# Edresson/VoiceSplit

Hardware: AMD Instinct MI355X
Metric: utterances/sec (3 s clips, B=64/GPU) fwd+bwd, channels-last bf16 activations / tape, bf16 MFMA, fp32 accumulate / statistics / master weights (higher is better)
Workload: dtype bf16 (conv activations and tape stored as bf16; bf16 MFMA operands in the convs, the LSTM / head contractions and the BPTT, f16 operands in the forward recurrence; fp32 accumulate, BatchNorm statistics, gate arithmetic / cell state, loss head, master weights)

## Files before the change

voicesplit_amd/csrc/nhwc_edge.hip:

```cpp
#include "vs_internal.h"

namespace {

typedef unsigned u4v __attribute__((ext_vector_type(4)));
typedef unsigned u2v __attribute__((ext_vector_type(2)));

__device__ __forceinline__ float bf_lo(unsigned u) { return __uint_as_float(u << 16); }
__device__ __forceinline__ float bf_hi(unsigned u) { return __uint_as_float(u & 0xffff0000u); }

template <int NV>
__device__ __forceinline__ void fold_channel_sums(float (&v)[NV][8], double* __restrict__ stats, float* lds ,
                                                  unsigned* turn = nullptr) {
  const int lane = threadIdx.x & 63, wave = threadIdx.x >> 6;
#pragma unroll
  for (int q = 0; q < NV; ++q)
#pragma unroll
    for (int j = 0; j < 8; ++j) {
      float s = v[q][j];
      s += __shfl_xor(s, 8, 64);
      s += __shfl_xor(s, 16, 64);
      s += __shfl_xor(s, 32, 64);
      if (lane < 8) lds[(wave * NV + q) * 64 + lane * 8 + j] = s;
    }
  __syncthreads();
// ... 264 lines not shown
    for (int q = 0; q < 4; ++q) {
      const float z0 = bf_lo(v[q]), z1 = bf_hi(v[q]);
      const float d0 = bf_lo(g[q]) * nhwc_act_grad<ACT>(fmaf(z0, sc[2 * q], sh[2 * q]));
      const float d1 = bf_hi(g[q]) * nhwc_act_grad<ACT>(fmaf(z1, sc[2 * q + 1], sh[2 * q + 1]));
      o[q] = vs_pack_bf16(fmaf(cA[2 * q], d0, fmaf(cB[2 * q], z0, cC[2 * q])),
                          fmaf(cA[2 * q + 1], d1, fmaf(cB[2 * q + 1], z1, cC[2 * q + 1])));
    }
    return o;
  };
  long long i = (long long)blockIdx.x * 256 + threadIdx.x;
  for (; i + stride < npieces; i += 2 * stride) {
    const u4v g0 = __builtin_nontemporal_load(da + i), v0 = __builtin_nontemporal_load(z + i);
    const u4v g1 = __builtin_nontemporal_load(da + i + stride), v1 = __builtin_nontemporal_load(z + i + stride);
    __builtin_nontemporal_store(apply(g0, v0), dz + i);
    __builtin_nontemporal_store(apply(g1, v1), dz + i + stride);
  }
  if (i < npieces) __builtin_nontemporal_store(apply(__builtin_nontemporal_load(da + i), __builtin_nontemporal_load(z + i)), dz + i);
}

template <int ACT>
__global__ __launch_bounds__(256)
void nhwc_bn_bwd_first_kernel(const u4v* __restrict__ da, const u4v* __restrict__ z, const float* __restrict__ x,
                              long long npix, int F, const float* __restrict__ scale, const float* __restrict__ shift,
                              const float* __restrict__ coef, double* __restrict__ acc_out ) {
  __shared__ float red[4 * 7 * 64];
  const int piece = threadIdx.x & 7;
  float sc[8], sh[8], cA[8], cB[8], cC[8], acc[7][8];
#pragma unroll
  for (int j = 0; j < 8; ++j) {
    const int c = piece * 8 + j;
    sc[j] = scale[c]; sh[j] = shift[c]; cA[j] = coef[c]; cB[j] = coef[64 + c]; cC[j] = coef[128 + c];
#pragma unroll
    for (int k = 0; k < 7; ++k) acc[k][j] = 0.f;
  }
  const long long stride = (long long)gridDim.x * 32;
  const int sr = (int)(stride % F);
  long long p = (long long)blockIdx.x * 32 + (threadIdx.x >> 3);
  int f = (int)(p % F);
  for (; p < npix; p += stride, f += sr) {
    if (f >= F) f -= F;
    float xv[7];
    gather_x7(x + (p - f), f, F, piece, xv);
    const u4v g = __builtin_nontemporal_load(da + p * 8 + piece), v = __builtin_nontemporal_load(z + p * 8 + piece);
#pragma unroll
    for (int q = 0; q < 4; ++q) {
#pragma unroll
      for (int e = 0; e < 2; ++e) {
        const int j = 2 * q + e;
        const float zv = e ? bf_hi(v[q]) : bf_lo(v[q]);
        const float dy = (e ? bf_hi(g[q]) : bf_lo(g[q])) * nhwc_act_grad<ACT>(fmaf(zv, sc[j], sh[j]));
        const float dzv = fmaf(cA[j], dy, fmaf(cB[j], zv, cC[j]));
#pragma unroll
        for (int k = 0; k < 7; ++k) acc[k][j] = fmaf(dzv, xv[k], acc[k][j]);
      }
    }
  }
  const int lane = threadIdx.x & 63, wave = threadIdx.x >> 6;
#pragma unroll
  for (int k = 0; k < 7; ++k)
#pragma unroll
    for (int j = 0; j < 8; ++j) {
      float s = acc[k][j];
      s += __shfl_xor(s, 8, 64);
      s += __shfl_xor(s, 16, 64);
      s += __shfl_xor(s, 32, 64);
      if (lane < 8) red[(wave * 7 + k) * 64 + lane * 8 + j] = s;
    }
  __syncthreads();
  for (int i = threadIdx.x; i < 7 * 64; i += 256) {
    const int k = i / 64, c = i - k * 64;
    atomicAdd(acc_out + c * 7 + k, (double)(red[(0 * 7 + k) * 64 + c] + red[(1 * 7 + k) * 64 + c] + red[(2 * 7 + k) * 64 + c] + red[(3 * 7 + k) * 64 + c]));
  }
}

__global__ void nhwc_cvt_f64_f32_kernel(const double* __restrict__ src, float* __restrict__ dst, int n) {
  const int i = blockIdx.x * blockDim.x + threadIdx.x;
  if (i < n) dst[i] = (float)src[i];
}

struct LastBwdBn {
  const u4v* z;
  const float *scale, *shift, *mean, *invstd;
  double* stats;
  unsigned* turn;
};

template <int ACT>
__device__ __forceinline__ void nhwc_act_both(float y, float& a, float& d) {
  if (ACT == VS_ACT_MISH) {
    const float u = __builtin_amdgcn_exp2f(fminf(y, 20.0f) * 1.44269504088896340736f);
    const float n = u * (u + 2.0f);
    const float r = __builtin_amdgcn_rcpf(n + 2.0f);
    a = y * (n * r);
    const float dd = r * fmaf(4.0f * y * r, u * (u + 1.0f), n);
    d = y > 20.0f ? 1.0f : dd;
  } else if (ACT == VS_ACT_RELU) {
    a = fmaxf(y, 0.0f);
    d = y > 0.0f ? 1.0f : 0.0f;
  } else {
    a = y;
    d = 1.0f;
  }
}

template <int ACT>
__device__ __forceinline__ void nhwc_act_both2(vs_f32x2 y, vs_f32x2& a, vs_f32x2& d) {
  if (ACT == VS_ACT_MISH) {
    const vs_f32x2 yc = {fminf(y.x, 20.0f), fminf(y.y, 20.0f)};
    const vs_f32x2 e = yc * 1.44269504088896340736f;
    const vs_f32x2 u = {__builtin_amdgcn_exp2f(e.x), __builtin_amdgcn_exp2f(e.y)};
    const vs_f32x2 n = u * (u + 2.0f);
    const vs_f32x2 dn = n + 2.0f;
    const vs_f32x2 r = {__builtin_amdgcn_rcpf(dn.x), __builtin_amdgcn_rcpf(dn.y)};
    a = y * (n * r);
    d = r * __builtin_elementwise_fma((yc * 4.0f) * r, __builtin_elementwise_fma(u, u, u), n);
  } else if (ACT == VS_ACT_RELU) {
    a = vs_f32x2{fmaxf(y.x, 0.0f), fmaxf(y.y, 0.0f)};
    d = vs_f32x2{y.x > 0.0f ? 1.0f : 0.0f, y.y > 0.0f ? 1.0f : 0.0f};
  } else {
    a = y;
    d = vs_f32x2{1.0f, 1.0f};
  }
}

template <int DYACT, bool RECOMP = false>
__global__ __launch_bounds__(256)
void nhwc_conv_last_bwd_kernel(const float* __restrict__ dz8, const float* __restrict__ w, const u4v* __restrict__ a7,
                               u4v* __restrict__ din, float* __restrict__ part, long long npix, int F, LastBwdBn bn) {
  __shared__ float red[4 * 8 * 64];
  const int piece = threadIdx.x & 7;
  vs_f32x2 wr[8][4], acc[8][4];
  vs_f32x2 sc[4], sh[4], mu[4], is[4], bacc[2][4];
#pragma unroll
  for (int co = 0; co < 8; ++co)
#pragma unroll
    for (int q = 0; q < 4; ++q) {
      wr[co][q] = vs_f32x2{w[co * 64 + piece * 8 + 2 * q], w[co * 64 + piece * 8 + 2 * q + 1]};
      acc[co][q] = vs_f32x2{0.f, 0.f};
    }
  if (DYACT >= 0) {
#pragma unroll
    for (int q = 0; q < 4; ++q) {
      const int c = piece * 8 + 2 * q;
      sc[q] = vs_f32x2{bn.scale[c], bn.scale[c + 1]}; sh[q] = vs_f32x2{bn.shift[c], bn.shift[c + 1]};
      mu[q] = vs_f32x2{bn.mean[c], bn.mean[c + 1]}; is[q] = vs_f32x2{bn.invstd[c], bn.invstd[c + 1]};
      bacc[0][q] = vs_f32x2{0.f, 0.f}; bacc[1][q] = vs_f32x2{0.f, 0.f};
    }
  }
  const long long stride = (long long)gridDim.x * 32;
  const int sr = (int)(stride % F);
  const long long sq = stride / F;
  long long p = (long long)blockIdx.x * 32 + (threadIdx.x >> 3);
  long long row = p / F;
  int f = (int)(p - row * F);
  struct In { float d[8]; u4v zv, av; };
  auto fetch = [&](long long pq, long long rq, int fq, In& in) {
    const float* dzr = dz8 + rq * 8 * F + fq;
#pragma unroll
    for (int co = 0; co < 8; ++co) in.d[co] = dzr[(size_t)co * F];
    if (DYACT >= 0) in.zv = __builtin_nontemporal_load(bn.z + pq * 8 + piece);
    if (!RECOMP) in.av = __builtin_nontemporal_load(a7 + pq * 8 + piece);
  };
  In cur, nxt;
  cur.zv = cur.av = nxt.zv = nxt.av = u4v{0u, 0u, 0u, 0u};
  if (p < npix) fetch(p, row, f, cur);
  for (; p < npix; p += stride) {
    int fn = f + sr;
    long long rown = row + sq;
    if (fn >= F) { fn -= F; ++rown; }
    const long long pn = p + stride;
    if (pn < npix) fetch(pn, rown, fn, nxt);
    vs_f32x2 zf[4], dact[4];
    u4v av = cur.av;
    if (DYACT >= 0) {
#pragma unroll
      for (int q = 0; q < 4; ++q) {
        zf[q] = vs_f32x2{bf_lo(cur.zv[q]), bf_hi(cur.zv[q])};
        vs_f32x2 aq;
        nhwc_act_both2<(DYACT >= 0 ? DYACT : VS_ACT_NONE)>(__builtin_elementwise_fma(zf[q], sc[q], sh[q]), aq, dact[q]);
        if (RECOMP) av[q] = vs_pack_bf16(aq.x, aq.y);
      }
    }
    vs_f32x2 g[4];
#pragma unroll
    for (int q = 0; q < 4; ++q) g[q] = vs_f32x2{0.f, 0.f};
#pragma unroll
    for (int co = 0; co < 8; ++co) {
      const vs_f32x2 dd = {cur.d[co], cur.d[co]};
#pragma unroll
      for (int q = 0; q < 4; ++q) {
        g[q] = __builtin_elementwise_fma(wr[co][q], dd, g[q]);
        acc[co][q] = __builtin_elementwise_fma(dd, vs_f32x2{bf_lo(av[q]), bf_hi(av[q])}, acc[co][q]);
      }
    }
    if (DYACT >= 0) {
#pragma unroll
      for (int q = 0; q < 4; ++q) {
        g[q] *= dact[q];
        bacc[0][q] += g[q];
        bacc[1][q] = __builtin_elementwise_fma(g[q], (zf[q] - mu[q]) * is[q], bacc[1][q]);
      }
    }
    __builtin_nontemporal_store(u4v{vs_pack_bf16(g[0].x, g[0].y), vs_pack_bf16(g[1].x, g[1].y), vs_pack_bf16(g[2].x, g[2].y), vs_pack_bf16(g[3].x, g[3].y)},
                                din + p * 8 + piece);
    cur = nxt;
    f = fn;
    row = rown;
  }
  if (DYACT >= 0) {
    float b8[2][8];
#pragma unroll
    for (int q = 0; q < 4; ++q) {
      b8[0][2 * q] = bacc[0][q].x; b8[0][2 * q + 1] = bacc[0][q].y;
      b8[1][2 * q] = bacc[1][q].x; b8[1][2 * q + 1] = bacc[1][q].y;
    }
    fold_channel_sums<2>(b8, bn.stats, red, bn.turn);
    __syncthreads();
  }
  const int lane = threadIdx.x & 63, wave = threadIdx.x >> 6;
#pragma unroll
  for (int co = 0; co < 8; ++co)
#pragma unroll
    for (int j = 0; j < 8; ++j) {
      float s = (j & 1) ? acc[co][j >> 1].y : acc[co][j >> 1].x;
      s += __shfl_xor(s, 8, 64);
      s += __shfl_xor(s, 16, 64);
      s += __shfl_xor(s, 32, 64);
      if (lane < 8) red[(wave * 8 + co) * 64 + lane * 8 + j] = s;
    }
  __syncthreads();
  for (int i = threadIdx.x; i < 512; i += 256)
    part[(size_t)blockIdx.x * 512 + i] = red[i] + red[512 + i] + red[1024 + i] + red[1536 + i];
}

constexpr int kMomN = 7 + 28;

__global__ __launch_bounds__(256)
void nhwc_first_moments_kernel(const float* __restrict__ x, long long npix, int F, double* __restrict__ mom, unsigned* turn) {
  __shared__ float red[4][kMomN];
  float acc[kMomN];
#pragma unroll
  for (int i = 0; i < kMomN; ++i) acc[i] = 0.f;
  const long long stride = (long long)gridDim.x * 256;
  for (long long p = (long long)blockIdx.x * 256 + threadIdx.x; p < npix; p += stride) {
    const int f = (int)(p % F);
    const float* xr = x + (p - f);
    float xv[7];
#pragma unroll
    for (int k = 0; k < 7; ++k) {
      const int ff = f + k - 3;
      xv[k] = (ff >= 0 && ff < F) ? xr[ff] : 0.f;
    }
    int i = 7;
#pragma unroll
    for (int k = 0; k < 7; ++k) {
      acc[k] += xv[k];
#pragma unroll
      for (int k2 = k; k2 < 7; ++k2) { acc[i] = fmaf(xv[k], xv[k2], acc[i]); ++i; }
    }
  }
  const int lane = threadIdx.x & 63, wave = threadIdx.x >> 6;
#pragma unroll
  for (int i = 0; i < kMomN; ++i) {
    float v = acc[i];
#pragma unroll
    for (int o = 32; o > 0; o >>= 1) v += __shfl_xor(v, o, 64);
    if (lane == 0) red[wave][i] = v;
  }
  __syncthreads();
  const unsigned slot = blockIdx.x % VS_BN_STAT_SLOTS, rank_in_slot = blockIdx.x / VS_BN_STAT_SLOTS;
  unsigned* my_turn = turn ? turn + VS_TURN_SLOT + slot : nullptr;
  if (turn) mom += (size_t)slot * 64;
  vs_turn_begin(my_turn, rank_in_slot);
  if (threadIdx.x < kMomN) atomicAdd(mom + threadIdx.x, (double)red[0][threadIdx.x] + (double)red[1][threadIdx.x] + (double)red[2][threadIdx.x] + (double)red[3][threadIdx.x]);
  vs_turn_end(my_turn, rank_in_slot, (gridDim.x - slot + VS_BN_STAT_SLOTS - 1) / VS_BN_STAT_SLOTS);
}

__global__ void fold_moment_slots_kernel(const double* __restrict__ slots, double* __restrict__ mom) {
  if (threadIdx.x >= kMomN) return;
  double v = 0.0;
  for (int k = 0; k < VS_BN_STAT_SLOTS; ++k) v += slots[(size_t)k * 64 + threadIdx.x];
  mom[threadIdx.x] = v;
}

__device__ __forceinline__ double mom_R(const double* mom, int k, int k2) {
  if (k > k2) { const int t = k; k = k2; k2 = t; }
  return mom[7 + k * 7 - k * (k - 1) / 2 + (k2 - k)];
}

__global__ void nhwc_first_stats_kernel(const double* __restrict__ mom, const float* __restrict__ w, const float* __restrict__ bias,
                                        double count, double* __restrict__ stats) {
  const int c = threadIdx.x;
  if (c >= 64) return;
  const double b = bias[c];
  double ws = 0.0, q = 0.0;
  for (int k = 0; k < 7; ++k) {
    ws += (double)w[c * 7 + k] * mom[k];
    for (int k2 = 0; k2 < 7; ++k2) q += (double)w[c * 7 + k] * (double)w[c * 7 + k2] * mom_R(mom, k, k2);
  }
  stats[2 * c] = ws + count * b;
  stats[2 * c + 1] = q + 2.0 * b * ws + count * b * b;
}

template <int ACT>
__device__ __forceinline__ vs_f32x2 nhwc_act_grad2(vs_f32x2 y) {
  if (ACT == VS_ACT_RELU) return vs_f32x2{y.x > 0.f ? 1.f : 0.f, y.y > 0.f ? 1.f : 0.f};
  if (ACT == VS_ACT_MISH) {
    const vs_f32x2 yc = {fminf(y.x, 20.0f), fminf(y.y, 20.0f)};
    const vs_f32x2 e = yc * 1.44269504088896340736f;
    const vs_f32x2 u = {__builtin_amdgcn_exp2f(e.x), __builtin_amdgcn_exp2f(e.y)};
    const vs_f32x2 n = u * (u + 2.0f);
    const vs_f32x2 d = n + 2.0f;
    const vs_f32x2 r = {__builtin_amdgcn_rcpf(d.x), __builtin_amdgcn_rcpf(d.y)};
    const vs_f32x2 t = __builtin_elementwise_fma(u, u, u);
    return r * __builtin_elementwise_fma((yc * 4.0f) * r, t, n);
  }
  return vs_f32x2{1.f, 1.f};
}

template <int ACT>
__global__ __launch_bounds__(256)
void nhwc_first_bwd_kernel(const u4v* __restrict__ da, const float* __restrict__ x, const float* __restrict__ w, const float* __restrict__ bias,
                           long long npix, int F, const float* __restrict__ scale, const float* __restrict__ shift,
                           const float* __restrict__ mean, const float* __restrict__ invstd, double* __restrict__ acc_out ,
                           unsigned* turn) {
  __shared__ float red[4 * 9 * 64];
  const int piece = threadIdx.x & 7;
  vs_f32x2 wr[4][7], bs[4], sc[4], sh[4], mu[4], is[4], acc[9][4];
#pragma unroll
  for (int q = 0; q < 4; ++q) {
    const int c0 = piece * 8 + 2 * q;
    bs[q] = vs_f32x2{bias[c0], bias[c0 + 1]};
    sc[q] = vs_f32x2{scale[c0], scale[c0 + 1]};
    sh[q] = vs_f32x2{shift[c0], shift[c0 + 1]};
    mu[q] = vs_f32x2{mean[c0], mean[c0 + 1]};
    is[q] = vs_f32x2{invstd[c0], invstd[c0 + 1]};
#pragma unroll
    for (int k = 0; k < 7; ++k) wr[q][k] = vs_f32x2{w[c0 * 7 + k], w[(c0 + 1) * 7 + k]};
#pragma unroll
    for (int k = 0; k < 9; ++k) acc[k][q] = vs_f32x2{0.f, 0.f};
  }
  const long long stride = (long long)gridDim.x * 32;
  const int sr = (int)(stride % F);
  long long p = (long long)blockIdx.x * 32 + (threadIdx.x >> 3);
  int f = (int)(p % F);
  auto process = [&](float mine, const u4v& g) {
    float xv[7];
    exchange_x7(mine, xv);
#pragma unroll
    for (int q = 0; q < 4; ++q) {
      vs_f32x2 zv = bs[q];
#pragma unroll
      for (int k = 0; k < 7; ++k) zv = __builtin_elementwise_fma(wr[q][k], vs_f32x2{xv[k], xv[k]}, zv);
      const vs_f32x2 dy = vs_f32x2{bf_lo(g[q]), bf_hi(g[q])} * nhwc_act_grad2<ACT>(__builtin_elementwise_fma(zv, sc[q], sh[q]));
      acc[0][q] += dy;
      acc[1][q] = __builtin_elementwise_fma(dy, (zv - mu[q]) * is[q], acc[1][q]);
#pragma unroll
      for (int k = 0; k < 7; ++k) acc[2 + k][q] = __builtin_elementwise_fma(dy, vs_f32x2{xv[k], xv[k]}, acc[2 + k][q]);
    }
  };
  float mine = 0.f;
  u4v g = {0u, 0u, 0u, 0u};
  if (p < npix) {
    mine = load_x7(x + (p - f), f, F, piece);
    g = __builtin_nontemporal_load(da + p * 8 + piece);
  }
  for (; p < npix; p += stride) {
    int fn = f + sr;
    if (fn >= F) fn -= F;
    const long long pn = p + stride;
    float mine_next = 0.f;
    u4v g_next = {0u, 0u, 0u, 0u};
    if (pn < npix) {
      mine_next = load_x7(x + (pn - fn), fn, F, piece);
      g_next = __builtin_nontemporal_load(da + pn * 8 + piece);
    }
    process(mine, g);
    mine = mine_next;
    g = g_next;
    f = fn;
  }
  const int lane = threadIdx.x & 63, wave = threadIdx.x >> 6;
#pragma unroll
  for (int k = 0; k < 9; ++k)
#pragma unroll
    for (int j = 0; j < 8; ++j) {
      float s = (j & 1) ? acc[k][j >> 1].y : acc[k][j >> 1].x;
      s += __shfl_xor(s, 8, 64);
      s += __shfl_xor(s, 16, 64);
      s += __shfl_xor(s, 32, 64);
      if (lane < 8) red[(wave * 9 + k) * 64 + lane * 8 + j] = s;
    }
  __syncthreads();
  const unsigned slot = blockIdx.x % VS_BN_STAT_SLOTS, rank_in_slot = blockIdx.x / VS_BN_STAT_SLOTS;
  unsigned* my_turn = turn ? turn + VS_TURN_SLOT + slot : nullptr;
  double* dst = turn ? acc_out + (size_t)slot * 576 : acc_out;
  vs_turn_begin(my_turn, rank_in_slot);
  for (int i = threadIdx.x; i < 9 * 64; i += 256) {
    const int k = i / 64, c = i - k * 64;
    atomicAdd(dst + c * 9 + k, (double)(red[(0 * 9 + k) * 64 + c] + red[(1 * 9 + k) * 64 + c] + red[(2 * 9 + k) * 64 + c] + red[(3 * 9 + k) * 64 + c]));
  }
  vs_turn_end(my_turn, rank_in_slot, (gridDim.x - slot + VS_BN_STAT_SLOTS - 1) / VS_BN_STAT_SLOTS);
}

__global__ void fold_slots_f64_kernel(const double* __restrict__ slots, int nslots, int n, double* __restrict__ out) {
  const int i = blockIdx.x * blockDim.x + threadIdx.x;
  if (i >= n) return;
  double v = 0.0;
  for (int k = 0; k < nslots; ++k) v += slots[(size_t)k * n + i];
  out[i] = v;
}

__global__ void nhwc_first_bwd_finalize_kernel(const double* __restrict__ acc , const double* __restrict__ mom,
                                               const float* __restrict__ w, const float* __restrict__ bias, const float* __restrict__ scale,
                                               const float* __restrict__ mean, const float* __restrict__ invstd, double count, int train,
                                               float* __restrict__ dgamma, float* __restrict__ dbeta, float* __restrict__ dbias, float* __restrict__ dw) {
  const int c = threadIdx.x;
  if (c >= 64) return;
  const double sdy = acc[c * 9], sdyx = acc[c * 9 + 1];
  dgamma[c] = (float)sdyx;
  dbeta[c] = (float)sdy;
  const double cA = scale[c];
  double cB = 0.0, cC = 0.0;
  if (train) {
    cB = -cA * (double)invstd[c] * sdyx / count;
    cC = -cA * sdy / count - cB * (double)mean[c];
  }
  dbias[c] = train ? 0.f : (float)(cA * sdy);
  const double b = bias[c];
  for (int k = 0; k < 7; ++k) {
    double zx = b * mom[k];
    for (int k2 = 0; k2 < 7; ++k2) zx += (double)w[c * 7 + k2] * mom_R(mom, k2, k);
    dw[c * 7 + k] = (float)(cA * acc[c * 9 + 2 + k] + cB * zx + cC * mom[k]);
  }
}

int stream_blocks(long long items_per_block_sweep, long long total, long long cap = 2048) {
  long long nb = (total + items_per_block_sweep - 1) / items_per_block_sweep;
  if (nb > cap) nb = cap;
  return nb < 1 ? 1 : (int)nb;
}
int stream_blocks_wide(long long items_per_block_sweep, long long total) {
  long long nb = (total + items_per_block_sweep - 1) / items_per_block_sweep;
  if (nb > (1LL << 24)) nb = 1LL << 24;
  return nb < 1 ? 1 : (int)nb;
}

}

int vs_nhwc_conv_first_impl(const float* x, const float* w, const float* scale, const float* shift, void* out,
                            int B, int T, int F, int act, double* bn_stats, hipStream_t stream, const float* bias) {
  VS_REQUIRE(x && w && scale && shift && out, "nhwc conv_first: NULL argument");
  VS_REQUIRE(B > 0 && T > 0 && F > 0, "nhwc conv_first: bad shape");
  const long long npix = (long long)B * T * F;
  const dim3 grid(stream_blocks(32, npix, (bn_stats && g_vs_turn) ? 2048 : 8192)), block(256);
  unsigned short* o = reinterpret_cast<unsigned short*>(out);
  if (bn_stats) {
    VS_REQUIRE(act == VS_ACT_NONE, "nhwc conv_first: fused statistics go with no activation");
    hipLaunchKernelGGL((nhwc_conv_first_kernel<VS_ACT_NONE, true>), grid, block, 0, stream, x, w, scale, shift, o, npix, F, bn_stats, bias);
  } else if (act == VS_ACT_NONE) hipLaunchKernelGGL((nhwc_conv_first_kernel<VS_ACT_NONE, false>), grid, block, 0, stream, x, w, scale, shift, o, npix, F, nullptr, bias);
  else if (act == VS_ACT_MISH) hipLaunchKernelGGL((nhwc_conv_first_kernel<VS_ACT_MISH, false>), grid, block, 0, stream, x, w, scale, shift, o, npix, F, nullptr, bias);
  else if (act == VS_ACT_RELU) hipLaunchKernelGGL((nhwc_conv_first_kernel<VS_ACT_RELU, false>), grid, block, 0, stream, x, w, scale, shift, o, npix, F, nullptr, bias);
  else VS_REQUIRE(false, "nhwc conv_first: unsupported activation %d", act);
  VS_LAUNCH_CHECK();
  return 0;
}

int vs_nhwc_first_moments_impl(const float* x, int B, int T, int F, double* mom, hipStream_t stream, double* det_slots, int mom_is_zero) {
  VS_REQUIRE(x && mom && B > 0 && T > 0 && F > 0, "nhwc first_moments: bad argument");
  const long long npix = (long long)B * T * F;
  if (!mom_is_zero) VS_CHECK_HIP(hipMemsetAsync(mom, 0, sizeof(double) * kMomN, stream));
  long long nb = (npix + 256 * 16 - 1) / (256 * 16);
  if (nb > 512) nb = 512;
  unsigned* turn = det_slots ? g_vs_turn : nullptr;
  if (turn) {
    VS_CHECK_HIP(hipMemsetAsync(det_slots, 0, sizeof(double) * VS_BN_STAT_SLOTS * 64, stream));
  }
  hipLaunchKernelGGL(nhwc_first_moments_kernel, dim3((unsigned)(nb < 1 ? 1 : nb)), dim3(256), 0, stream, x, npix, F, turn ? det_slots : mom, turn);
  if (turn) hipLaunchKernelGGL(fold_moment_slots_kernel, dim3(1), dim3(64), 0, stream, det_slots, mom);
  VS_LAUNCH_CHECK();
  return 0;
}

int vs_nhwc_first_stats_impl(const double* mom, const float* w, const float* bias, double count, double* stats, hipStream_t stream) {
  VS_REQUIRE(mom && w && bias && stats && count > 0, "nhwc first_stats: bad argument");
  hipLaunchKernelGGL(nhwc_first_stats_kernel, dim3(1), dim3(64), 0, stream, mom, w, bias, count, stats);
  VS_LAUNCH_CHECK();
  return 0;
}

int vs_nhwc_first_bwd_impl(const void* da, const float* x, const float* w, const float* bias, int B, int T, int F, int act, int train,
                           const float* scale, const float* shift, const float* mean, const float* invstd,
                           float* dgamma, float* dbeta, float* dbias, float* dw, double* scratch, hipStream_t stream, const double* moments, double* det_slots) {
  VS_REQUIRE(da && x && w && bias && scale && shift && mean && invstd && dgamma && dbeta && dbias && dw && scratch, "nhwc first_bwd: NULL argument");
  VS_REQUIRE(B > 0 && T > 0 && F > 0, "nhwc first_bwd: bad shape");
  const long long npix = (long long)B * T * F;
  double* acc = scratch;
  VS_CHECK_HIP(hipMemsetAsync(acc, 0, sizeof(double) * 64 * 9, stream));
  const double* mom = moments;
  if (!mom) {
    if (int rc = vs_nhwc_first_moments_impl(x, B, T, F, scratch + 64 * 9, stream)) return rc;
    mom = scratch + 64 * 9;
  }
  const u4v* g = reinterpret_cast<const u4v*>(da);
  unsigned* turn = det_slots ? g_vs_turn : nullptr;
  const dim3 grid(stream_blocks(32, npix)), block(256);
  double* sums = turn ? det_slots : acc;
  if (turn) VS_CHECK_HIP(hipMemsetAsync(det_slots, 0, sizeof(double) * VS_BN_STAT_SLOTS * 576, stream));
  if (act == VS_ACT_MISH) hipLaunchKernelGGL(nhwc_first_bwd_kernel<VS_ACT_MISH>, grid, block, 0, stream, g, x, w, bias, npix, F, scale, shift, mean, invstd, sums, turn);
  else if (act == VS_ACT_RELU) hipLaunchKernelGGL(nhwc_first_bwd_kernel<VS_ACT_RELU>, grid, block, 0, stream, g, x, w, bias, npix, F, scale, shift, mean, invstd, sums, turn);
  else if (act == VS_ACT_NONE) hipLaunchKernelGGL(nhwc_first_bwd_kernel<VS_ACT_NONE>, grid, block, 0, stream, g, x, w, bias, npix, F, scale, shift, mean, invstd, sums, turn);
  else VS_REQUIRE(false, "nhwc first_bwd: unsupported activation %d", act);
  if (turn) hipLaunchKernelGGL(fold_slots_f64_kernel, dim3(3), dim3(192), 0, stream, det_slots, VS_BN_STAT_SLOTS, 576, acc);
  hipLaunchKernelGGL(nhwc_first_bwd_finalize_kernel, dim3(1), dim3(64), 0, stream, acc, mom, w, bias, scale, mean, invstd, (double)npix, train,
                     dgamma, dbeta, dbias, dw);
  VS_LAUNCH_CHECK();
  return 0;
}

int vs_nhwc_bn_apply_impl(const void* z, void* a, long long npix, int act, const float* scale, const float* shift, hipStream_t stream) {
  VS_REQUIRE(z && a && scale && shift && npix > 0, "nhwc bn_apply: bad argument");
  const long long npieces = npix * 8;
  const dim3 grid(stream_blocks_wide(512, npieces)), block(256);
  const u4v* zi = reinterpret_cast<const u4v*>(z);
  u4v* ao = reinterpret_cast<u4v*>(a);
  if (act == VS_ACT_MISH) hipLaunchKernelGGL(nhwc_bn_apply_kernel<VS_ACT_MISH>, grid, block, 0, stream, zi, ao, scale, shift, npieces);
  else if (act == VS_ACT_RELU) hipLaunchKernelGGL(nhwc_bn_apply_kernel<VS_ACT_RELU>, grid, block, 0, stream, zi, ao, scale, shift, npieces);
  else if (act == VS_ACT_NONE) hipLaunchKernelGGL(nhwc_bn_apply_kernel<VS_ACT_NONE>, grid, block, 0, stream, zi, ao, scale, shift, npieces);
  else VS_REQUIRE(false, "nhwc bn_apply: unsupported activation %d", act);
  VS_LAUNCH_CHECK();
  return 0;
}

int vs_nhwc_conv_last_impl(const void* in, const float* w, const float* scale, const float* shift, float* out,
                           int B, int T, int F, int act, hipStream_t stream, double* bn_stats,
                           const float* pre_scale, const float* pre_shift, int pre_act, void* rows_bf16, int Kp) {
  VS_REQUIRE(in && w && scale && shift && (out || rows_bf16), "nhwc conv_last: NULL argument");
  VS_REQUIRE(!rows_bf16 || (!bn_stats && !pre_scale && Kp >= 8 * F), "nhwc conv_last: the row form is the plain eval layer's (Kp = %d)", Kp);
  unsigned short* rb = reinterpret_cast<unsigned short*>(rows_bf16);
  VS_REQUIRE(!pre_scale == !pre_shift, "nhwc conv_last: pre_scale and pre_shift come together");
  VS_REQUIRE(B > 0 && T > 0 && F > 0, "nhwc conv_last: bad shape");
  const long long nrows = (long long)B * T;
  const long long nblk = nrows * ((F + 15) / 16);
  const dim3 grid(stream_blocks(4, nblk, (bn_stats && g_vs_turn) ? 2048 : 8192)), block(256);
  const unsigned short* i = reinterpret_cast<const unsigned short*>(in);
  if (pre_scale) {
    VS_REQUIRE(act == VS_ACT_NONE, "nhwc conv_last: the pre-activation form writes the unactivated output");
    VS_REQUIRE(pre_act == VS_ACT_MISH || pre_act == VS_ACT_RELU, "nhwc conv_last: pre-activation %d", pre_act);
#define VS_LAST_PRE(ST_, PRE_) hipLaunchKernelGGL((nhwc_conv_last_kernel<VS_ACT_NONE, ST_, PRE_>), grid, block, 0, stream, i, w, scale, shift, out, nrows, F, bn_stats, pre_scale, pre_shift, \
                                                  (unsigned short*)nullptr, 0, ST_ ? g_vs_turn : (unsigned*)nullptr)
    if (bn_stats) { if (pre_act == VS_ACT_MISH) VS_LAST_PRE(true, VS_ACT_MISH); else VS_LAST_PRE(true, VS_ACT_RELU); }
    else { if (pre_act == VS_ACT_MISH) VS_LAST_PRE(false, VS_ACT_MISH); else VS_LAST_PRE(false, VS_ACT_RELU); }
#undef VS_LAST_PRE
    VS_LAUNCH_CHECK();
    return 0;
  }
  if (bn_stats) {
    VS_REQUIRE(act == VS_ACT_NONE, "nhwc conv_last: statistics are those of the unactivated output");
    hipLaunchKernelGGL((nhwc_conv_last_kernel<VS_ACT_NONE, true>), grid, block, 0, stream, i, w, scale, shift, out, nrows, F, bn_stats,
                       (const float*)nullptr, (const float*)nullptr, (unsigned short*)nullptr, 0, g_vs_turn);
    VS_LAUNCH_CHECK();
    return 0;
  }
  const float* nof = nullptr;
  if (act == VS_ACT_MISH) hipLaunchKernelGGL(nhwc_conv_last_kernel<VS_ACT_MISH>, grid, block, 0, stream, i, w, scale, shift, out, nrows, F, (double*)nullptr, nof, nof, rb, Kp);
  else if (act == VS_ACT_RELU) hipLaunchKernelGGL(nhwc_conv_last_kernel<VS_ACT_RELU>, grid, block, 0, stream, i, w, scale, shift, out, nrows, F, (double*)nullptr, nof, nof, rb, Kp);
  else if (act == VS_ACT_NONE) hipLaunchKernelGGL(nhwc_conv_last_kernel<VS_ACT_NONE>, grid, block, 0, stream, i, w, scale, shift, out, nrows, F, (double*)nullptr, nof, nof, rb, Kp);
  else VS_REQUIRE(false, "nhwc conv_last: unsupported activation %d", act);
  VS_LAUNCH_CHECK();
  return 0;
}

int vs_nhwc_bn_act_bwd_impl(const void* da, const void* z, void* dz, long long npix, int act, int train,
                            const float* scale, const float* shift, const float* mean, const float* invstd,
                            float* dgamma, float* dbeta, float* dbias, double* stats , float* coef,
                            hipStream_t stream, int beside_wgrad) {
  VS_REQUIRE(da && z && dz && scale && shift && mean && invstd && stats && coef && npix > 0, "nhwc bn_act_bwd: bad argument");
  const long long npieces = npix * 8;
  int nb = stream_blocks(512, npieces);
  if (beside_wgrad) {
    const int want = 256;
    if (want < nb) nb = want;
  }
  const dim3 grid(nb), block(256);
  const u4v* g = reinterpret_cast<const u4v*>(da);
  const u4v* zz = reinterpret_cast<const u4v*>(z);
  VS_CHECK_HIP(hipMemsetAsync(stats, 0, sizeof(double) * VS_BN_STAT_SLOTS * 128, stream));
  if (act == VS_ACT_MISH) hipLaunchKernelGGL(nhwc_bn_bwd_stats_kernel<VS_ACT_MISH>, grid, block, 0, stream, g, zz, npieces, scale, shift, mean, invstd, stats);
  else if (act == VS_ACT_RELU) hipLaunchKernelGGL(nhwc_bn_bwd_stats_kernel<VS_ACT_RELU>, grid, block, 0, stream, g, zz, npieces, scale, shift, mean, invstd, stats);
  else if (act == VS_ACT_NONE) hipLaunchKernelGGL(nhwc_bn_bwd_stats_kernel<VS_ACT_NONE>, grid, block, 0, stream, g, zz, npieces, scale, shift, mean, invstd, stats);
  else VS_REQUIRE(false, "nhwc bn_act_bwd: unsupported activation %d", act);
  if (int rc = vs_bn_bwd_finalize_impl(stats, VS_BN_STAT_SLOTS, (double)npix, train, 64, scale, mean, invstd, dgamma, dbeta, dbias, coef, stream)) return rc;
  u4v* o = reinterpret_cast<u4v*>(dz);
  if (act == VS_ACT_MISH) hipLaunchKernelGGL(nhwc_bn_bwd_apply_kernel<VS_ACT_MISH>, grid, block, 0, stream, g, zz, o, npieces, scale, shift, coef);
  else if (act == VS_ACT_RELU) hipLaunchKernelGGL(nhwc_bn_bwd_apply_kernel<VS_ACT_RELU>, grid, block, 0, stream, g, zz, o, npieces, scale, shift, coef);
  else hipLaunchKernelGGL(nhwc_bn_bwd_apply_kernel<VS_ACT_NONE>, grid, block, 0, stream, g, zz, o, npieces, scale, shift, coef);
  VS_LAUNCH_CHECK();
  return 0;
}

int vs_nhwc_bn_bwd_from_dy_impl(const void* dy, const void* z, void* dz, long long npix, int train,
                                const float* scale, const float* mean, const float* invstd,
                                float* dgamma, float* dbeta, float* dbias, double* stats, float* coef, hipStream_t stream, int rezero_doubles,
                                int beside_wgrad) {
  VS_REQUIRE(dy && z && dz && scale && mean && invstd && stats && coef && npix > 0, "nhwc bn_bwd_from_dy: bad argument");
  const long long npieces = npix * 8;
  int nb = beside_wgrad ? stream_blocks(512, npieces) : stream_blocks_wide(512, npieces);
  if (beside_wgrad) {
    const int want = 256;
    if (want < nb) nb = want;
  }
  const dim3 grid(nb), block(256);
  if (int rc = vs_bn_bwd_finalize_impl(stats, VS_BN_STAT_SLOTS, (double)npix, train, 64, scale, mean, invstd, dgamma, dbeta, dbias, coef, stream,
                                       rezero_doubles)) return rc;
  hipLaunchKernelGGL(nhwc_bn_bwd_apply_kernel<VS_ACT_NONE>, grid, block, 0, stream, reinterpret_cast<const u4v*>(dy), reinterpret_cast<const u4v*>(z),
                     reinterpret_cast<u4v*>(dz), npieces, scale, scale, coef);
  VS_LAUNCH_CHECK();
  return 0;
}

int vs_nhwc_bn_bwd_first_from_dy_impl(const void* dy, const void* z, const float* x, int B, int T, int F, int train,
                                      const float* scale, const float* mean, const float* invstd,
                                      float* dgamma, float* dbeta, float* dbias, float* dw, double* stats, float* coef, double* acc ,
                                      hipStream_t stream) {
  VS_REQUIRE(dy && z && x && dw && stats && coef && acc, "nhwc bn_bwd_first_from_dy: NULL argument");
  const long long npix = (long long)B * T * F;
  if (int rc = vs_bn_bwd_finalize_impl(stats, VS_BN_STAT_SLOTS, (double)npix, train, 64, scale, mean, invstd, dgamma, dbeta, dbias, coef, stream)) return rc;
  VS_CHECK_HIP(hipMemsetAsync(acc, 0, sizeof(double) * 448, stream));
  const dim3 grid(stream_blocks(32, npix)), block(256);
  hipLaunchKernelGGL(nhwc_bn_bwd_first_kernel<VS_ACT_NONE>, grid, block, 0, stream, reinterpret_cast<const u4v*>(dy), reinterpret_cast<const u4v*>(z),
                     x, npix, F, scale, scale, coef, acc);
  hipLaunchKernelGGL(nhwc_cvt_f64_f32_kernel, dim3(2), dim3(256), 0, stream, acc, dw, 448);
  VS_LAUNCH_CHECK();
  return 0;
}

int vs_nhwc_bn_act_bwd_first_impl(const void* da, const void* z, const float* x, int B, int T, int F, int act, int train,
                                  const float* scale, const float* shift, const float* mean, const float* invstd,
                                  float* dgamma, float* dbeta, float* dbias, float* dw, double* stats, float* coef, double* acc ,
                                  hipStream_t stream) {
  VS_REQUIRE(da && z && x && dw && stats && coef && acc, "nhwc bn_act_bwd_first: NULL argument");
  const long long npix = (long long)B * T * F, npieces = npix * 8;
  const u4v* g = reinterpret_cast<const u4v*>(da);
  const u4v* zz = reinterpret_cast<const u4v*>(z);
  {
    const dim3 grid(stream_blocks(512, npieces)), block(256);
    VS_CHECK_HIP(hipMemsetAsync(stats, 0, sizeof(double) * VS_BN_STAT_SLOTS * 128, stream));
    if (act == VS_ACT_MISH) hipLaunchKernelGGL(nhwc_bn_bwd_stats_kernel<VS_ACT_MISH>, grid, block, 0, stream, g, zz, npieces, scale, shift, mean, invstd, stats);
    else if (act == VS_ACT_RELU) hipLaunchKernelGGL(nhwc_bn_bwd_stats_kernel<VS_ACT_RELU>, grid, block, 0, stream, g, zz, npieces, scale, shift, mean, invstd, stats);
    else if (act == VS_ACT_NONE) hipLaunchKernelGGL(nhwc_bn_bwd_stats_kernel<VS_ACT_NONE>, grid, block, 0, stream, g, zz, npieces, scale, shift, mean, invstd, stats);
    else VS_REQUIRE(false, "nhwc bn_act_bwd_first: unsupported activation %d", act);
  }
  if (int rc = vs_bn_bwd_finalize_impl(stats, VS_BN_STAT_SLOTS, (double)npix, train, 64, scale, mean, invstd, dgamma, dbeta, dbias, coef, stream)) return rc;
  VS_CHECK_HIP(hipMemsetAsync(acc, 0, sizeof(double) * 448, stream));
  const dim3 grid(stream_blocks(32, npix)), block(256);
  if (act == VS_ACT_MISH) hipLaunchKernelGGL(nhwc_bn_bwd_first_kernel<VS_ACT_MISH>, grid, block, 0, stream, g, zz, x, npix, F, scale, shift, coef, acc);
  else if (act == VS_ACT_RELU) hipLaunchKernelGGL(nhwc_bn_bwd_first_kernel<VS_ACT_RELU>, grid, block, 0, stream, g, zz, x, npix, F, scale, shift, coef, acc);
  else hipLaunchKernelGGL(nhwc_bn_bwd_first_kernel<VS_ACT_NONE>, grid, block, 0, stream, g, zz, x, npix, F, scale, shift, coef, acc);
  hipLaunchKernelGGL(nhwc_cvt_f64_f32_kernel, dim3(2), dim3(256), 0, stream, acc, dw, 448);
  VS_LAUNCH_CHECK();
  return 0;
}

int vs_nhwc_conv_last_bwd_impl(const float* dz8, const float* w, const void* a7, void* din, float* part, float* dw,
                               int B, int T, int F, const void* z7, int act, const float* bn_scale, const float* bn_shift,
                               const float* bn_mean, const float* bn_invstd, double* bn_stats, hipStream_t stream) {
  VS_REQUIRE(dz8 && w && din && part && dw, "nhwc conv_last_bwd: NULL argument");
  VS_REQUIRE(a7 || z7, "nhwc conv_last_bwd: a7 may only be NULL in the dy form (it is then recomputed from z7)");
  VS_REQUIRE(!z7 || (bn_scale && bn_shift && bn_mean && bn_invstd && bn_stats), "nhwc conv_last_bwd: the dy form needs the BatchNorm constants and statistics slots");
  const long long npix = (long long)B * T * F;
  long long nb = (npix + 31) / 32;
  if (nb > VS_NHWC_LAST_BWD_BLOCKS) nb = VS_NHWC_LAST_BWD_BLOCKS;
  const LastBwdBn bn{reinterpret_cast<const u4v*>(z7), bn_scale, bn_shift, bn_mean, bn_invstd, bn_stats, z7 ? g_vs_turn : nullptr};
  const dim3 grid((unsigned)nb), block(256);
  const u4v* a = reinterpret_cast<const u4v*>(a7);
  u4v* o = reinterpret_cast<u4v*>(din);
  if (!z7) hipLaunchKernelGGL(nhwc_conv_last_bwd_kernel<-1>, grid, block, 0, stream, dz8, w, a, o, part, npix, F, bn);
  else if (act == VS_ACT_MISH && !a7) hipLaunchKernelGGL((nhwc_conv_last_bwd_kernel<VS_ACT_MISH, true>), grid, block, 0, stream, dz8, w, a, o, part, npix, F, bn);
  else if (act == VS_ACT_RELU && !a7) hipLaunchKernelGGL((nhwc_conv_last_bwd_kernel<VS_ACT_RELU, true>), grid, block, 0, stream, dz8, w, a, o, part, npix, F, bn);
  else if (act == VS_ACT_MISH) hipLaunchKernelGGL(nhwc_conv_last_bwd_kernel<VS_ACT_MISH>, grid, block, 0, stream, dz8, w, a, o, part, npix, F, bn);
  else if (act == VS_ACT_RELU) hipLaunchKernelGGL(nhwc_conv_last_bwd_kernel<VS_ACT_RELU>, grid, block, 0, stream, dz8, w, a, o, part, npix, F, bn);
  else VS_REQUIRE(false, "nhwc conv_last_bwd: dy form for activation %d", act);
  VS_LAUNCH_CHECK();
  return vs_reduce_partials_impl(part, (int)nb, 512, dw, stream);
}

namespace {

typedef _Float16 h8v __attribute__((ext_vector_type(8)));
typedef _Float16 h2v __attribute__((ext_vector_type(2)));

__global__ void nhwc_first_plan_kernel(const unsigned* __restrict__ amax_in, int n_amax, const float* __restrict__ w, const float* __restrict__ scale,
                                       const float* __restrict__ shift, float* __restrict__ out_scale2, int nco, int taps) {
  const int c = threadIdx.x;
  unsigned mb = 0;
  for (int i = c; i < n_amax; i += 64) mb = amax_in[i] > mb ? amax_in[i] : mb;
#pragma unroll
  for (int o = 32; o > 0; o >>= 1) { const unsigned other = __shfl_xor(mb, o, 64); mb = other > mb ? other : mb; }
  float bound = 0.3125f;
  if (c < nco) {
    float l1 = 0.f;
    for (int k = 0; k < taps; ++k) l1 += fabsf(w[c * taps + k]);
    bound = fmaxf(fabsf(scale[c]) * l1 * __uint_as_float(mb) + fabsf(shift[c]), 0.3125f);
  }
#pragma unroll
  for (int o = 32; o > 0; o >>= 1) bound = fmaxf(bound, __shfl_xor(bound, o, 64));
  if (c == 0) {
    float s = 1.f, si = 1.f;
    if (bound > 0.f && bound < 3.0e38f) {
      int e = 0;
      (void)frexpf(bound, &e);
      int k = 15 - e;
      k = k > 100 ? 100 : (k < -100 ? -100 : k);
      s = ldexpf(1.f, k);
      si = ldexpf(1.f, -k);
    }
    out_scale2[0] = s;
    out_scale2[1] = si;
  }
}

__global__ __launch_bounds__(256)
void absmax_any_kernel(const float* __restrict__ x, long long n, unsigned* __restrict__ amax) {
  __shared__ float red[4];
  float m = 0.f;
  for (long long i = (long long)blockIdx.x * blockDim.x + threadIdx.x; i < n; i += (long long)gridDim.x * blockDim.x) m = fmaxf(m, fabsf(x[i]));
#pragma unroll
  for (int o = 32; o > 0; o >>= 1) m = fmaxf(m, __shfl_xor(m, o, 64));
  if ((threadIdx.x & 63) == 0) red[threadIdx.x >> 6] = m;
  __syncthreads();
  if (threadIdx.x == 0) {
    m = fmaxf(fmaxf(red[0], red[1]), fmaxf(red[2], red[3]));
    if (m > 0.f) atomicMax(amax, __float_as_uint(m));
  }
}

template <int ACT>
__global__ __launch_bounds__(256)
void nhwc_conv_first_split_kernel(const float* __restrict__ x, const float* __restrict__ w, const float* __restrict__ scale,
                                  const float* __restrict__ shift, const float* __restrict__ out_scale2, unsigned short* __restrict__ out_hi,
                                  unsigned short* __restrict__ out_lo, unsigned* __restrict__ amax_out, long long npix, int F) {
  const int piece = threadIdx.x & 7;
  vs_f32x2 wr[4][7], sc[4], sh[4];
#pragma unroll
  for (int q = 0; q < 4; ++q) {
    const int c0 = piece * 8 + 2 * q;
    sc[q] = vs_f32x2{scale[c0], scale[c0 + 1]};
    sh[q] = vs_f32x2{shift[c0], shift[c0 + 1]};
#pragma unroll
    for (int k = 0; k < 7; ++k) wr[q][k] = vs_f32x2{w[c0 * 7 + k], w[(c0 + 1) * 7 + k]};
  }
  const float sy = out_scale2[0];
  float am = 0.f;
  const long long stride = (long long)gridDim.x * 32;
  const int sr = (int)(stride % F);
  long long p = (long long)blockIdx.x * 32 + (threadIdx.x >> 3);
  int f = (int)(p % F);
  float mine = p < npix ? load_x7(x + (p - f), f, F, piece) : 0.f;
  for (; p < npix; p += stride) {
    int fn = f + sr;
    if (fn >= F) fn -= F;
    const long long pn = p + stride;
    const float mine_next = pn < npix ? load_x7(x + (pn - fn), fn, F, piece) : 0.f;
    float xv[7];
    exchange_x7(mine, xv);
    mine = mine_next;
    f = fn;
    u4v ph, pl;
#pragma unroll
    for (int q = 0; q < 4; ++q) {
      vs_f32x2 s2 = {0.f, 0.f};
#pragma unroll
      for (int k = 0; k < 7; ++k) s2 = __builtin_elementwise_fma(wr[q][k], vs_f32x2{xv[k], xv[k]}, s2);
      vs_f32x2 y = vs_act_fast2<ACT>(__builtin_elementwise_fma(s2, sc[q], sh[q]));
      am = fmaxf(am, fmaxf(fabsf(y.x), fabsf(y.y)));
      y = y * sy;
      const unsigned hb = __builtin_bit_cast(unsigned, __builtin_amdgcn_cvt_pkrtz(y.x, y.y));
      const h2v h = __builtin_bit_cast(h2v, hb);
      ph[q] = hb;
      pl[q] = __builtin_bit_cast(unsigned, __builtin_amdgcn_cvt_pkrtz(y.x - (float)h[0], y.y - (float)h[1]));
    }
    __builtin_nontemporal_store(ph, reinterpret_cast<u4v*>(out_hi + p * 64 + piece * 8));
    __builtin_nontemporal_store(pl, reinterpret_cast<u4v*>(out_lo + p * 64 + piece * 8));
  }
  vs_absmax_commit(am, amax_out);
}

template <int ACT, bool ROWS>
__global__ __launch_bounds__(256)
void nhwc_conv_last_split_kernel(const unsigned short* __restrict__ in_hi, const unsigned short* __restrict__ in_lo, const float* __restrict__ in_scale2,
                                 const float* __restrict__ w, const float* __restrict__ scale, const float* __restrict__ shift,
                                 float* __restrict__ out, long long nrows, int F,
                                 unsigned short* __restrict__ row_hi, unsigned short* __restrict__ row_lo, int Kp, const float* __restrict__ out_scale2) {
  const int lane = threadIdx.x & 63, n = lane & 15, g = lane >> 4;
  float wv[2][8], wmax = 0.f;
#pragma unroll
  for (int kc = 0; kc < 2; ++kc)
#pragma unroll
    for (int j = 0; j < 8; ++j) {
      wv[kc][j] = w[(n & 7) * 64 + kc * 32 + g * 8 + j];
      wmax = fmaxf(wmax, fabsf(wv[kc][j]));
    }
#pragma unroll
  for (int o = 32; o > 0; o >>= 1) wmax = fmaxf(wmax, __shfl_xor(wmax, o, 64));
  float sw = 1.f, swi = 1.f;
  if (wmax > 0.f && wmax < 3.0e38f) {
    int e = 0;
    (void)frexpf(wmax, &e);
    sw = ldexpf(1.f, 10 - e);
    swi = ldexpf(1.f, e - 10);
  }
  h8v wh[2], wl[2];
#pragma unroll
  for (int kc = 0; kc < 2; ++kc)
// ... 150 lines not shown
```

Measured before the change: 1445.

## Recast first-layer conv backward reductions as fp32 MFMA tiles

Rewrites the first (7-tap, 64-channel) conv+BN backward kernel so the per-pixel pre-activation recompute and the dy·x weight-gradient reductions run as 16x16x4 fp32 MFMA ops over 16-pixel tiles per wave, with double-buffered tile loads. It folds BN scale/shift into the weights, drops the separate dy·x̂ accumulator and reconstructs it in the finalize kernel from the weight sums, and uses a raw v_min for the Mish clamp. The aim is to cut VALU FMA work and register pressure in a bandwidth/ALU-bound reduction. In exchange it adds MFMA identity-transpose tricks and more complex edge handling, and the reconstructed dgamma path changes the floating-point summation order.

```diff
diff --git a/voicesplit_amd/csrc/nhwc_edge.hip b/voicesplit_amd/csrc/nhwc_edge.hip
--- a/voicesplit_amd/csrc/nhwc_edge.hip
+++ b/voicesplit_amd/csrc/nhwc_edge.hip
@@ -590,11 +590,16 @@
   stats[2 * c + 1] = q + 2.0 * b * ws + count * b * b;
 }
 
+__device__ __forceinline__ float vs_min_raw(float a, float b) {
+  float r;
+  asm("v_min_f32_e32 %0, %1, %2" : "=v"(r) : "s"(b), "v"(a));
+  return r;
+}
 template <int ACT>
 __device__ __forceinline__ vs_f32x2 nhwc_act_grad2(vs_f32x2 y) {
   if (ACT == VS_ACT_RELU) return vs_f32x2{y.x > 0.f ? 1.f : 0.f, y.y > 0.f ? 1.f : 0.f};
   if (ACT == VS_ACT_MISH) {
-    const vs_f32x2 yc = {fminf(y.x, 20.0f), fminf(y.y, 20.0f)};
+    const vs_f32x2 yc = {vs_min_raw(y.x, 20.0f), vs_min_raw(y.y, 20.0f)};
     const vs_f32x2 e = yc * 1.44269504088896340736f;
     const vs_f32x2 u = {__builtin_amdgcn_exp2f(e.x), __builtin_amdgcn_exp2f(e.y)};
     const vs_f32x2 n = u * (u + 2.0f);
@@ -606,87 +611,137 @@
   return vs_f32x2{1.f, 1.f};
 }
 
+typedef float f4v __attribute__((ext_vector_type(4)));
+
+struct FirstBwdTile {
+  u2v d[4];
+  float xa0, xa1;
+  int fa, rem;
+};
+
+template <bool FULL>
+__device__ __forceinline__ void first_bwd_load(FirstBwdTile& tl, const u2v* __restrict__ da, const float* __restrict__ x, long long base ,
+                                               long long npix, int F, int fa, int n, int g, int ma) {
+  const float* xw = x + base;
+  const u2v* dw = da + base * 16;
+  const int rem = FULL ? 16 : (int)(npix - base);
+  const int f0 = fa + g - 3, f1 = fa + g + 1;
+  const bool pv = FULL || ma < rem;
+  const bool v0 = pv && (unsigned)f0 < (unsigned)F, v1 = pv && g < 3 && f1 < F;
+  tl.xa0 = xw[v0 ? ma + g - 3 : 0];
+  tl.xa1 = xw[v1 ? ma + g + 1 : 0];
+  tl.fa = fa;
+  tl.rem = rem;
+#pragma unroll
+  for (int j = 0; j < 4; ++j) {
+    const int q = g + 4 * j;
+    if (FULL) {
+      tl.d[j] = __builtin_nontemporal_load(dw + (q * 16 + n));
+    } else {
+      const u2v dv = __builtin_nontemporal_load(dw + (q < rem ? q * 16 + n : n));
+      tl.d[j] = q < rem ? dv : u2v{0u, 0u};
+    }
+  }
+}
+
+__device__ __forceinline__ void first_bwd_taps(const FirstBwdTile& tl, int F, int g, int ma, float& xa0, float& xa1) {
+  const bool pv = ma < tl.rem;
+  xa0 = (pv && (unsigned)(tl.fa + g - 3) < (unsigned)F) ? tl.xa0 : 0.f;
+  xa1 = (pv && g < 3 && tl.fa + g + 1 < F) ? tl.xa1 : (g == 3 ? 1.f : 0.f);
+}
+
 template <int ACT>
 __global__ __launch_bounds__(256)
-void nhwc_first_bwd_kernel(const u4v* __restrict__ da, const float* __restrict__ x, const float* __restrict__ w, const float* __restrict__ bias,
+void nhwc_first_bwd_kernel(const u2v* __restrict__ da, const float* __restrict__ x, const float* __restrict__ w, const float* __restrict__ bias,
                            long long npix, int F, const float* __restrict__ scale, const float* __restrict__ shift,
-                           const float* __restrict__ mean, const float* __restrict__ invstd, double* __restrict__ acc_out ,
-                           unsigned* turn) {
-  __shared__ float red[4 * 9 * 64];
-  const int piece = threadIdx.x & 7;
-  vs_f32x2 wr[4][7], bs[4], sc[4], sh[4], mu[4], is[4], acc[9][4];
-#pragma unroll
-  for (int q = 0; q < 4; ++q) {
-    const int c0 = piece * 8 + 2 * q;
-    bs[q] = vs_f32x2{bias[c0], bias[c0 + 1]};
-    sc[q] = vs_f32x2{scale[c0], scale[c0 + 1]};
-    sh[q] = vs_f32x2{shift[c0], shift[c0 + 1]};
-    mu[q] = vs_f32x2{mean[c0], mean[c0 + 1]};
-    is[q] = vs_f32x2{invstd[c0], invstd[c0 + 1]};
-#pragma unroll
-    for (int k = 0; k < 7; ++k) wr[q][k] = vs_f32x2{w[c0 * 7 + k], w[(c0 + 1) * 7 + k]};
-#pragma unroll
-    for (int k = 0; k < 9; ++k) acc[k][q] = vs_f32x2{0.f, 0.f};
-  }
-  const long long stride = (long long)gridDim.x * 32;
+                           double* __restrict__ acc_out , unsigned* turn) {
+  __shared__ float red[4 * 8 * 64];
+  const int lane = threadIdx.x & 63, wave = __builtin_amdgcn_readfirstlane(threadIdx.x >> 6);
+  const int n = lane & 15, g = lane >> 4;
+  float bw[4][2];
+#pragma unroll
+  for (int t = 0; t < 4; ++t) {
+    const int c = 4 * n + t;
+    bw[t][0] = scale[c] * w[c * 7 + g];
+    bw[t][1] = g < 3 ? scale[c] * w[c * 7 + 4 + g] : fmaf(scale[c], bias[c], shift[c]);
+  }
+  const float id0 = n == g ? 1.f : 0.f, id1 = n == 4 + g ? 1.f : 0.f;
+  f4v S[4];
+#pragma unroll
+  for (int t = 0; t < 4; ++t) S[t] = f4v{0.f, 0.f, 0.f, 0.f};
+  const long long stride = (long long)gridDim.x * 64;
   const int sr = (int)(stride % F);
-  long long p = (long long)blockIdx.x * 32 + (threadIdx.x >> 3);
-  int f = (int)(p % F);
-  auto process = [&](float mine, const u4v& g) {
-    float xv[7];
-    exchange_x7(mine, xv);
-#pragma unroll
-    for (int q = 0; q < 4; ++q) {
-      vs_f32x2 zv = bs[q];
-#pragma unroll
-      for (int k = 0; k < 7; ++k) zv = __builtin_elementwise_fma(wr[q][k], vs_f32x2{xv[k], xv[k]}, zv);
-      const vs_f32x2 dy = vs_f32x2{bf_lo(g[q]), bf_hi(g[q])} * nhwc_act_grad2<ACT>(__builtin_elementwise_fma(zv, sc[q], sh[q]));
-      acc[0][q] += dy;
-      acc[1][q] = __builtin_elementwise_fma(dy, (zv - mu[q]) * is[q], acc[1][q]);
-#pragma unroll
-      for (int k = 0; k < 7; ++k) acc[2 + k][q] = __builtin_elementwise_fma(dy, vs_f32x2{xv[k], xv[k]}, acc[2 + k][q]);
-    }
+  long long p0 = ((long long)blockIdx.x * 4 + wave) * 16;
+  const long long full_end = npix - 16;
+  const int ma = 4 * (n & 3) + (n >> 2);
+  int fa = (int)((p0 + ma) % F);
+  auto load_whole = [&](long long base, FirstBwdTile& tl) {
+    first_bwd_load<true>(tl, da, x, base, npix, F, fa, n, g, ma);
+    fa += sr;
+    if (fa >= F) fa -= F;
+    __builtin_amdgcn_sched_barrier(0);
   };
-  float mine = 0.f;
-  u4v g = {0u, 0u, 0u, 0u};
-  if (p < npix) {
-    mine = load_x7(x + (p - f), f, F, piece);
-    g = __builtin_nontemporal_load(da + p * 8 + piece);
-  }
-  for (; p < npix; p += stride) {
-    int fn = f + sr;
-    if (fn >= F) fn -= F;
-    const long long pn = p + stride;
-    float mine_next = 0.f;
-    u4v g_next = {0u, 0u, 0u, 0u};
-    if (pn < npix) {
-      mine_next = load_x7(x + (pn - fn), fn, F, piece);
-      g_next = __builtin_nontemporal_load(da + pn * 8 + piece);
-    }
-    process(mine, g);
-    mine = mine_next;
-    g = g_next;
-    f = fn;
-  }
-  const int lane = threadIdx.x & 63, wave = threadIdx.x >> 6;
-#pragma unroll
-  for (int k = 0; k < 9; ++k)
-#pragma unroll
-    for (int j = 0; j < 8; ++j) {
-      float s = (j & 1) ? acc[k][j >> 1].y : acc[k][j >> 1].x;
-      s += __shfl_xor(s, 8, 64);
-      s += __shfl_xor(s, 16, 64);
-      s += __shfl_xor(s, 32, 64);
-      if (lane < 8) red[(wave * 9 + k) * 64 + lane * 8 + j] = s;
-    }
+  auto process = [&](const FirstBwdTile& tl) {
+    const f4v zero = {0.f, 0.f, 0.f, 0.f};
+    float xa0, xa1;
+    first_bwd_taps(tl, F, g, ma, xa0, xa1);
+    f4v xt = __builtin_amdgcn_mfma_f32_16x16x4f32(xa0, id0, zero, 0, 0, 0);
+    xt = __builtin_amdgcn_mfma_f32_16x16x4f32(xa1, id1, xt, 0, 0, 0);
+    f4v y[4];
+#pragma unroll
+    for (int t = 0; t < 4; ++t) {
+      y[t] = __builtin_amdgcn_mfma_f32_16x16x4f32(xa0, bw[t][0], zero, 0, 0, 0);
+      y[t] = __builtin_amdgcn_mfma_f32_16x16x4f32(xa1, bw[t][1], y[t], 0, 0, 0);
+    }
+#pragma unroll
+    for (int t = 0; t < 4; ++t) {
+#pragma unroll
+      for (int j = 0; j < 4; j += 2) {
+        const unsigned u0 = tl.d[j][t >> 1], u1 = tl.d[j + 1][t >> 1];
+        const vs_f32x2 gv = (t & 1) ? vs_f32x2{bf_hi(u0), bf_hi(u1)} : vs_f32x2{bf_lo(u0), bf_lo(u1)};
+        const vs_f32x2 dy = gv * nhwc_act_grad2<ACT>(vs_f32x2{y[t][j], y[t][j + 1]});
+        S[t] = __builtin_amdgcn_mfma_f32_16x16x4f32(dy.x, xt[j], S[t], 0, 0, 0);
+        S[t] = __builtin_amdgcn_mfma_f32_16x16x4f32(dy.y, xt[j + 1], S[t], 0, 0, 0);
+      }
+    }
+  };
+  FirstBwdTile ta, tb;
+  if (p0 <= full_end) {
+    load_whole(p0, ta);
+    while (p0 + stride <= full_end) {
+      load_whole(p0 + stride, tb);
+      process(ta);
+      p0 += stride;
+      if (p0 + stride > full_end) {
+        ta = tb;
+        break;
+      }
+      load_whole(p0 + stride, ta);
+      process(tb);
+      p0 += stride;
+    }
+    process(ta);
+    p0 += stride;
+  }
+  if (p0 < npix) {
+    first_bwd_load<false>(ta, da, x, p0, npix, F, fa, n, g, ma);
+    process(ta);
+  }
+  if (n < 8) {
+#pragma unroll
+    for (int t = 0; t < 4; ++t)
+#pragma unroll
+      for (int r = 0; r < 4; ++r) red[(wave * 8 + n) * 64 + 16 * g + 4 * r + t] = S[t][r];
+  }
   __syncthreads();
   const unsigned slot = blockIdx.x % VS_BN_STAT_SLOTS, rank_in_slot = blockIdx.x / VS_BN_STAT_SLOTS;
   unsigned* my_turn = turn ? turn + VS_TURN_SLOT + slot : nullptr;
   double* dst = turn ? acc_out + (size_t)slot * 576 : acc_out;
   vs_turn_begin(my_turn, rank_in_slot);
-  for (int i = threadIdx.x; i < 9 * 64; i += 256) {
+  for (int i = threadIdx.x; i < 8 * 64; i += 256) {
     const int k = i / 64, c = i - k * 64;
-    atomicAdd(dst + c * 9 + k, (double)(red[(0 * 9 + k) * 64 + c] + red[(1 * 9 + k) * 64 + c] + red[(2 * 9 + k) * 64 + c] + red[(3 * 9 + k) * 64 + c]));
+    atomicAdd(dst + c * 9 + (k < 7 ? 2 + k : 0),
+              (double)(red[(0 * 8 + k) * 64 + c] + red[(1 * 8 + k) * 64 + c] + red[(2 * 8 + k) * 64 + c] + red[(3 * 8 + k) * 64 + c]));
   }
   vs_turn_end(my_turn, rank_in_slot, (gridDim.x - slot + VS_BN_STAT_SLOTS - 1) / VS_BN_STAT_SLOTS);
 }
@@ -705,7 +760,10 @@
                                                float* __restrict__ dgamma, float* __restrict__ dbeta, float* __restrict__ dbias, float* __restrict__ dw) {
   const int c = threadIdx.x;
   if (c >= 64) return;
-  const double sdy = acc[c * 9], sdyx = acc[c * 9 + 1];
+  const double sdy = acc[c * 9];
+  double sdyx = ((double)bias[c] - (double)mean[c]) * sdy;
+  for (int k = 0; k < 7; ++k) sdyx += (double)w[c * 7 + k] * acc[c * 9 + 2 + k];
+  sdyx *= (double)invstd[c];
   dgamma[c] = (float)sdyx;
   dbeta[c] = (float)sdy;
   const double cA = scale[c];
@@ -790,14 +848,14 @@
     if (int rc = vs_nhwc_first_moments_impl(x, B, T, F, scratch + 64 * 9, stream)) return rc;
     mom = scratch + 64 * 9;
   }
-  const u4v* g = reinterpret_cast<const u4v*>(da);
+  const u2v* g = reinterpret_cast<const u2v*>(da);
   unsigned* turn = det_slots ? g_vs_turn : nullptr;
-  const dim3 grid(stream_blocks(32, npix)), block(256);
+  const dim3 grid(stream_blocks(64, npix)), block(256);
   double* sums = turn ? det_slots : acc;
   if (turn) VS_CHECK_HIP(hipMemsetAsync(det_slots, 0, sizeof(double) * VS_BN_STAT_SLOTS * 576, stream));
-  if (act == VS_ACT_MISH) hipLaunchKernelGGL(nhwc_first_bwd_kernel<VS_ACT_MISH>, grid, block, 0, stream, g, x, w, bias, npix, F, scale, shift, mean, invstd, sums, turn);
-  else if (act == VS_ACT_RELU) hipLaunchKernelGGL(nhwc_first_bwd_kernel<VS_ACT_RELU>, grid, block, 0, stream, g, x, w, bias, npix, F, scale, shift, mean, invstd, sums, turn);
-  else if (act == VS_ACT_NONE) hipLaunchKernelGGL(nhwc_first_bwd_kernel<VS_ACT_NONE>, grid, block, 0, stream, g, x, w, bias, npix, F, scale, shift, mean, invstd, sums, turn);
+  if (act == VS_ACT_MISH) hipLaunchKernelGGL(nhwc_first_bwd_kernel<VS_ACT_MISH>, grid, block, 0, stream, g, x, w, bias, npix, F, scale, shift, sums, turn);
+  else if (act == VS_ACT_RELU) hipLaunchKernelGGL(nhwc_first_bwd_kernel<VS_ACT_RELU>, grid, block, 0, stream, g, x, w, bias, npix, F, scale, shift, sums, turn);
+  else if (act == VS_ACT_NONE) hipLaunchKernelGGL(nhwc_first_bwd_kernel<VS_ACT_NONE>, grid, block, 0, stream, g, x, w, bias, npix, F, scale, shift, sums, turn);
   else VS_REQUIRE(false, "nhwc first_bwd: unsupported activation %d", act);
   if (turn) hipLaunchKernelGGL(fold_slots_f64_kernel, dim3(3), dim3(192), 0, stream, det_slots, VS_BN_STAT_SLOTS, 576, acc);
   hipLaunchKernelGGL(nhwc_first_bwd_finalize_kernel, dim3(1), dim3(64), 0, stream, acc, mom, w, bias, scale, mean, invstd, (double)npix, train,
```

New measurement: 1454, median of 6. Within noise of the previous version (+0.7%).
